# AutonomousVehicleLaboratory/vision_semantic_segmentation

Measured on AMD Instinct MI355X. Metric: fused frames/sec/GPU (1920x1080 + 120k pts) + max|dlog-odds| vs ref, higher is better.
Workload: dtype f16 hi+lo split, MX-FP4 correction passes, fp32 accumulate

## Files before the change

vision_semantic_segmentation_amd/csrc/seg_bottleneck.hip:

```cpp
#include "seg_types.h"

namespace avl {
namespace {

constexpr int BT_H = 8, BT_W = 16;
constexpr int BH_W = BT_W + 2, BH_H = BT_H + 2;
constexpr int BN_HALO = BH_W * BH_H;
constexpr int BN_M1 = 12;
constexpr int BN_WIDTH = 128, BN_COUT = 256;
constexpr int XSLAB = 192 * 128;
constexpr int PLANE1 = 192 * 256;
constexpr int PLANE2 = 128 * 256;

struct BnArgs {
    const f16* x;
    const f16* x_lo;
    f16* out;
    f16* out_lo;
    const f16* w1;
    const f16* w2;
    const f16* w3;
    const float* b1;
    const float* b2;
    const float* b3;
    int H, W, in_ld, out_ld;
    int tiles_x, ntiles;
    int out_bytes;
};

template <int CIN, bool DS, bool T1LO>
struct BnLayout {
    static constexpr int NCH = CIN / 64;
    static constexpr int XTILE = NCH * XSLAB;
    static constexpr int XBYTES = (DS ? 2 : 1) * XTILE;
    static constexpr int T1LO_OFF = PLANE1;
    static constexpr int T2LO_OFF = T1LO ? PLANE1 : PLANE2;
    static constexpr int ABYTES = T1LO ? 2 * PLANE1 : 2 * PLANE2;
    static constexpr int LDS = XBYTES + ABYTES;
    static_assert(LDS <= 160 * 1024, "bottleneck tile does not fit the LDS");
};

typedef f16 h2v __attribute__((ext_vector_type(2)));
typedef unsigned u32x4 __attribute__((ext_vector_type(4)));

__device__ __forceinline__ float relu_f32(float v) { return __builtin_amdgcn_fmed3f(v, 0.f, 3.0e38f); }

__device__ __forceinline__ uint2 relu_pack4(f32x4 v) {
    const h2v z = {(f16)0.f, (f16)0.f};
    const h2v a = __builtin_elementwise_max(h2v{(f16)v[0], (f16)v[1]}, z), b = __builtin_elementwise_max(h2v{(f16)v[2], (f16)v[3]}, z);
    return make_uint2(__builtin_bit_cast(unsigned, a), __builtin_bit_cast(unsigned, b));
}

__device__ __forceinline__ unsigned lo_pair(unsigned hipk, float v0, float v1) {
    unsigned d;
    asm("v_fma_mixlo_f16 %0, -%1, 1.0, %2 op_sel_hi:[1,0,0]" : "=v"(d) : "v"(hipk), "v"(v0));
    asm("v_fma_mixhi_f16 %0, -%1, 1.0, %2 op_sel:[1,0,0] op_sel_hi:[1,0,0]" : "+v"(d) : "v"(hipk), "v"(v1));
    return d;
}

__device__ __forceinline__ void split4(const float (&v)[4], uint2& hi, uint2& lo) {
    const h2v a = {(f16)v[0], (f16)v[1]}, b = {(f16)v[2], (f16)v[3]};
    hi = make_uint2(__builtin_bit_cast(unsigned, a), __builtin_bit_cast(unsigned, b));
    lo = make_uint2(lo_pair(hi.x, v[0], v[1]), lo_pair(hi.y, v[2], v[3]));
}

template <int CIN, bool DS, bool T1LO, bool XLO, bool OLO>
__global__ void __launch_bounds__(512) k_bottleneck(BnArgs p) {
    typedef BnLayout<CIN, DS, T1LO> L;
    constexpr int KS1 = CIN / 32;
    constexpr int KS3 = 4 + (DS ? CIN / 32 : 0);
    extern __shared__ __attribute__((aligned(16))) char lds[];
    const int tid = threadIdx.x, lane = tid & 63;
    const int wave = __builtin_amdgcn_readfirstlane(tid >> 6);
    const int c = lane & 15, q = lane >> 4;
    const unsigned lds0 = lds_addr(lds);
    char* const A = lds + L::XBYTES;
// ... 242 lines not shown
                    __builtin_amdgcn_raw_buffer_store_b128(u32x4{h0.x, h0.y, h1.x, h1.y}, orsrc, ooff, 0, 0);
                }
            }
        }
        {
            constexpr int NTAIL = (DS ? BT_H : BT_H - 2) * (OLO ? 2 : 1);
            if (more) asm volatile("s_waitcnt vmcnt(%0)" ::"n"(NTAIL) : "memory");
        }
        __syncthreads();
    }
}

int device_cus() {
    static int n = 0;
    if (n == 0) {
        int dev = 0;
        hipDeviceProp_t prop;
        if (hipGetDevice(&dev) == hipSuccess && hipGetDeviceProperties(&prop, dev) == hipSuccess) n = prop.multiProcessorCount;
        if (n <= 0) n = 256;
    }
    return n;
}

template <int CIN, bool DS, bool T1LO, bool XLO, bool OLO>
int launch_bn(const BnArgs& a, int nimg, hipStream_t s) {
    typedef BnLayout<CIN, DS, T1LO> L;
    AVL_HIP_CHECK(hipFuncSetAttribute(reinterpret_cast<const void*>(&k_bottleneck<CIN, DS, T1LO, XLO, OLO>), hipFuncAttributeMaxDynamicSharedMemorySize, L::LDS));
    const int grid = a.ntiles < device_cus() ? a.ntiles : device_cus();
    hipLaunchKernelGGL((k_bottleneck<CIN, DS, T1LO, XLO, OLO>), dim3(grid, 1, nimg), dim3(512), L::LDS, s, a);
    AVL_LAUNCH_CHECK();
    return AVL_OK;
}

}

int validate_bottleneck(const avl_seg_op& op) {
    AVL_REQUIRE(op.dtype == AVL_F16, "fused bottleneck: AVL_F16 activations only");
    AVL_REQUIRE(op.groups == 32 && op.ksize == 3 && op.stride == 1 && op.dil == 1 && op.pad == 1, "fused bottleneck: 3x3, 32 groups, stride 1, dilation 1");
    AVL_REQUIRE(op.out_c == BN_COUT && op.in3_c == BN_WIDTH, "fused bottleneck: width %d -> %d output channels only (got %d -> %d)", BN_WIDTH, BN_COUT, op.in3_c, op.out_c);
    AVL_REQUIRE((op.in_c == 64 && op.w_layout == 1) || (op.in_c == 256 && op.w_layout == 0 && op.w_split == 0),
                "fused bottleneck: 64 input channels with the downsample folded in, or 256 with the identity residual and no t1 lo plane");
    AVL_REQUIRE(op.in_h == op.out_h && op.in_w == op.out_w && op.in_h > 0 && op.in_w > 0, "fused bottleneck: same-size output");
    AVL_REQUIRE(op.in_ld >= op.in_c && op.in_ld % 8 == 0 && op.out_ld >= op.out_c && op.out_ld % 8 == 0, "fused bottleneck: row strides");
    AVL_REQUIRE((long long)op.in_rows >= (long long)op.in_h * op.in_w * op_batch(op) && (long long)op.out_rows >= (long long)op.out_h * op.out_w * op_batch(op),
                "fused bottleneck: rows allocated");
    AVL_REQUIRE((long long)op.in_rows * op.in_ld * 2 < (1LL << 31) && (long long)op.out_rows * op.out_ld * 2 < (1LL << 31), "fused bottleneck: planes beyond 2 GB (32-bit offsets)");
    AVL_REQUIRE(op.in && op.out && op.weight && op.in2 && op.in3 && op.bias, "fused bottleneck: in, out, weight (conv1), in2 (conv2 weights), in3 (conv3 weights), bias");
    AVL_REQUIRE(((reinterpret_cast<uintptr_t>(op.in) | reinterpret_cast<uintptr_t>(op.in_lo) | reinterpret_cast<uintptr_t>(op.out) | reinterpret_cast<uintptr_t>(op.out_lo) |
                  reinterpret_cast<uintptr_t>(op.weight) | reinterpret_cast<uintptr_t>(op.in2) | reinterpret_cast<uintptr_t>(op.in3) | reinterpret_cast<uintptr_t>(op.bias)) & 15) == 0,
                "fused bottleneck: 16-byte aligned buffers");
    AVL_REQUIRE(!(op.in_c == 64 && op.in_lo), "fused bottleneck: the 64-channel variant takes a single-plane input");
    AVL_REQUIRE(op.in != op.out && op.in != op.out_lo, "fused bottleneck: not in place (tiles read their neighbours' pixels)");
    return AVL_OK;
}

int launch_bottleneck(const avl_seg_op& op, hipStream_t s) {
    BnArgs a;
    a.x = static_cast<const f16*>(op.in);
    a.x_lo = static_cast<const f16*>(op.in_lo);
    a.out = static_cast<f16*>(op.out);
    a.out_lo = static_cast<f16*>(op.out_lo);
    a.w1 = static_cast<const f16*>(op.weight);
    a.w2 = static_cast<const f16*>(op.in2);
    a.w3 = static_cast<const f16*>(op.in3);
    a.b1 = op.bias; a.b2 = op.bias + BN_WIDTH; a.b3 = op.bias + 2 * BN_WIDTH;
    a.H = op.in_h; a.W = op.in_w; a.in_ld = op.in_ld; a.out_ld = op.out_ld;
    a.tiles_x = (op.in_w + BT_W - 1) / BT_W;
    a.ntiles = a.tiles_x * ((op.in_h + BT_H - 1) / BT_H);
    a.out_bytes = (int)((long long)op.out_rows * op.out_ld * 2);
    const int variant = (op.in_c == 64 ? 4 + 2 * (op.w_split ? 1 : 0) : 2 * (a.x_lo ? 1 : 0)) + (a.out_lo ? 1 : 0);
    switch (variant) {
        case 0: return launch_bn<256, false, false, false, false>(a, op_batch(op), s);
        case 1: return launch_bn<256, false, false, false, true>(a, op_batch(op), s);
        case 2: return launch_bn<256, false, false, true, false>(a, op_batch(op), s);
        case 3: return launch_bn<256, false, false, true, true>(a, op_batch(op), s);
        case 4: return launch_bn<64, true, false, false, false>(a, op_batch(op), s);
        case 5: return launch_bn<64, true, false, false, true>(a, op_batch(op), s);
        case 6: return launch_bn<64, true, true, false, false>(a, op_batch(op), s);
        default: return launch_bn<64, true, true, false, true>(a, op_batch(op), s);
    }
}

}
```

vision_semantic_segmentation_amd/csrc/seg_gemm.hip:

```cpp
#include <cstdlib>
#include <cstring>
#include <type_traits>

#include "seg_types.h"

namespace avl {
namespace {

struct GemmArgs {
    const void* A;
    const void* W;
    const float* bias;
    const void* R;
    void* C;
    int lda, ldr, ldc;
    int M, N, K;
    int relu, out_f32;
    int ntiles;
    int nsub;
    long long a_lo_delta;
    const void* R_lo;
    void* C_lo;
};

// ... 439 lines not shown
    constexpr int LDS = 2 * (WM * 64 + WN * 64) * 128;
    AVL_HIP_CHECK(hipFuncSetAttribute(reinterpret_cast<const void*>(&k_gemm<T, WM, WN>),
                                      hipFuncAttributeMaxDynamicSharedMemorySize, LDS));
    hipLaunchKernelGGL((k_gemm<T, WM, WN>), dim3(mtiles * a.ntiles), dim3(WM * WN * 64), LDS, s, a);
    AVL_LAUNCH_CHECK();
    return AVL_OK;
}

struct MxArgs {
    GemmArgs g;
    const char* Aq[2];
    const char* As[2];
    const char* Wq[2];
    const char* Ws[2];
    int ldaq;
    long long a_srows, w_srows;
    char* Cq[2];
    char* Cs[2];
    int ldcq;
    long long c_srows;
    int nmx;
    const char* Rq;
    const char* Rs;
    int ldrq;
    long long r_srows;
    int nmb1;
    const void* A2;
    int lda2, ldaq2;
    const char* Aq2[2];
    const char* As2[2];
    long long a_srows2;
    int stagger;
};

__device__ __forceinline__ unsigned quantize_fp4_block(const float (&v)[16], unsigned (&q)[2]) {
    float amax = 0.f;
#pragma unroll
    for (int i = 0; i < 16; ++i) amax = fmaxf(amax, fabsf(v[i]));
    {
        const unsigned ab = __float_as_uint(amax);
        const auto r16 = __builtin_amdgcn_permlane16_swap(ab, ab, false, false);
        amax = __uint_as_float(max(r16[0], r16[1]));
    }
    const unsigned sbyte = mx_fp4_scale_byte(amax);
    const float scale = __uint_as_float(sbyte << 23);
    q[0] = q[1] = 0u;
#define AVL_FP4_PAIR(i)                                                                                  \
    q[0] = __builtin_amdgcn_cvt_scalef32_pk_fp4_f32(q[0], v[2 * (i)], v[2 * (i) + 1], scale, (i));        \
    q[1] = __builtin_amdgcn_cvt_scalef32_pk_fp4_f32(q[1], v[8 + 2 * (i)], v[8 + 2 * (i) + 1], scale, (i))
    AVL_FP4_PAIR(0); AVL_FP4_PAIR(1); AVL_FP4_PAIR(2); AVL_FP4_PAIR(3);
#undef AVL_FP4_PAIR
    return sbyte;
}

template <int IO, int MI>
__device__ __forceinline__ void mx_epilogue(const MxArgs& q, f32x4 (&acc)[MI][4], int nt, int mt, int wm, int wn, int fr, int kq) {
    typedef f16 H;
    typedef typename Half16<H>::v8 v8;
    constexpr int BM = 2 * MI * 16, BN = 256;
    const GemmArgs& p = q.g;
    const int nbase = nt * BN + wn * 64 + kq * 16;
    const bool ncol_ok = nbase + 16 <= p.N;
    const bool rsplit = p.R_lo != nullptr, csplit = p.C_lo != nullptr;
    const unsigned m0 = (unsigned)(mt * BM + wm * (MI * 16) + fr);
    const unsigned sc_r = (unsigned)(nbase >> 8) * (unsigned)q.r_srows * 8u + (unsigned)((nbase >> 5) & 7);
    const unsigned sc_c = (unsigned)(nbase >> 8) * (unsigned)q.c_srows * 8u + (unsigned)((nbase >> 5) & 7);
    v8 nr0 = {}, nr1 = {};
    uint2 npk = make_uint2(0u, 0u);
    unsigned nsb = 127u;
    auto load_res = [&](int mi) {
        const unsigned m = m0 + mi * 16;
        if (p.R && (int)m < p.M && ncol_ok) {
            const H* rp = static_cast<const H*>(p.R) + (m * (unsigned)p.ldr + (unsigned)nbase);
            nr0 = *reinterpret_cast<const v8*>(rp);
            nr1 = *reinterpret_cast<const v8*>(rp + 8);
            if (q.Rq) {
                npk = *reinterpret_cast<const uint2*>(q.Rq + (m * (unsigned)q.ldrq + (unsigned)(nbase / 2)));
                nsb = (unsigned char)q.Rs[sc_r + m * 8u];
            }
        }
    };
    load_res(0);
#pragma unroll
    for (int mi = 0; mi < MI; ++mi) {
        const unsigned m = m0 + mi * 16;
        const bool live = (int)m < p.M && ncol_ok;
// ... 744 lines not shown
```

vision_semantic_segmentation_amd/csrc/seg_types.h:

```cpp
#pragma once
#include <hip/hip_runtime.h>

#include "avl_common.h"

namespace avl {

typedef __bf16 bf16;
typedef __bf16 bf16x8 __attribute__((ext_vector_type(8)));
typedef _Float16 f16;
typedef _Float16 f16x8 __attribute__((ext_vector_type(8)));
typedef float f32x4 __attribute__((ext_vector_type(4)));
typedef float f32x8 __attribute__((ext_vector_type(8)));

template <typename T>
struct Vec8;

template <>
struct Vec8<bf16> {
    static __device__ __forceinline__ void load(const bf16* p, float (&v)[8]) {
        const bf16x8 x = *reinterpret_cast<const bf16x8*>(p);
#pragma unroll
        for (int i = 0; i < 8; ++i) v[i] = (float)x[i];
    }
    static __device__ __forceinline__ void store(bf16* p, const float (&v)[8]) {
// ... 73 lines not shown
}

__device__ __forceinline__ void glds16_saddr(const void* sbase, unsigned voff, unsigned lds_byte_addr) {
    unsigned keep;
    asm volatile(
        "s_mov_b32 %0, m0\n\t"
        "s_mov_b32 m0, %3\n\t"
        "s_nop 0\n\t"
        "global_load_lds_dwordx4 %1, %2\n\t"
        "s_mov_b32 m0, %0"
        : "=&s"(keep)
        : "v"(voff), "s"(sbase), "s"(lds_byte_addr)
        : "memory");
}

__device__ __forceinline__ void glds4_saddr(const void* sbase, unsigned voff, unsigned lds_byte_addr) {
    unsigned keep;
    asm volatile(
        "s_mov_b32 %0, m0\n\t"
        "s_mov_b32 m0, %3\n\t"
        "s_nop 0\n\t"
        "global_load_lds_dword %1, %2\n\t"
        "s_mov_b32 m0, %0"
        : "=&s"(keep)
        : "v"(voff), "s"(sbase), "s"(lds_byte_addr)
        : "memory");
}

__device__ __forceinline__ unsigned mx_fp4_scale_byte(float amax) {
    const unsigned ab = __float_as_uint(amax), e = ab >> 23;
    return (e >= 3u ? e - 2u : 1u) + ((ab & 0x7fffffu) > 0x500000u ? 1u : 0u);
}

__device__ __forceinline__ unsigned lds_addr(const void* p) {
    return (unsigned)(size_t)(const __attribute__((address_space(3))) void*)p;
}

inline int elem_size(int dtype) { return dtype == AVL_F32 ? 4 : 2; }

inline int op_batch(const avl_seg_op& op) { return op.batch > 1 ? op.batch : 1; }
template <typename T>
__device__ __forceinline__ T* image_base(T* p, long long pixels, long long ld) {
    return p ? p + (long long)blockIdx.z * pixels * ld : p;
}
inline bool is_half(int dtype) { return dtype == AVL_BF16 || dtype == AVL_F16; }

int launch_gemm(const avl_seg_op& op, hipStream_t s);
int validate_gemm(const avl_seg_op& op);
int launch_conv_op(const avl_seg_op& op, hipStream_t s);
int validate_conv_op(const avl_seg_op& op);
int launch_gconv_mfma(const avl_seg_op& op, hipStream_t s);
int validate_gconv_mfma(const avl_seg_op& op);
int launch_conv3x3(const avl_seg_op& op, hipStream_t s);
int validate_conv3x3(const avl_seg_op& op);
int launch_stem_mfma(const avl_seg_op& op, hipStream_t s);
int launch_stem_pre_f32(const avl_seg_op& op, hipStream_t s);
int launch_dwconv_k(const avl_seg_op& op, hipStream_t s);
int validate_dwconv_k(const avl_seg_op& op);
int launch_dwpw(const avl_seg_op& op, hipStream_t s);
int validate_dwpw(const avl_seg_op& op);
int launch_bottleneck(const avl_seg_op& op, hipStream_t s);
int validate_bottleneck(const avl_seg_op& op);

}
```

vision_semantic_segmentation_amd/network.py:

```python
import ctypes as C
import math

import numpy as np
import torch

from . import _lib

BN_EPS = 1e-5

OP_STEM, OP_MAXPOOL, OP_GEMM, OP_GCONV, OP_DWCONV, OP_BILINEAR, OP_GAP, OP_GEMV, OP_ARGMAX, OP_SUBSAMPLE, OP_DWPW, OP_BOTTLENECK = range(1, 13)
OP_NAMES = {1: "stem", 2: "maxpool", 3: "gemm", 4: "gconv", 5: "dwconv", 6: "bilinear", 7: "gap", 8: "gemv", 9: "argmax", 10: "subsample", 11: "dwpw",
            12: "bottleneck"}


class AvlSegOp(C.Structure):
    _fields_ = [
        ("kind", C.c_int32), ("dtype", C.c_int32),
        ("in_", C.c_void_p), ("in2", C.c_void_p), ("out", C.c_void_p), ("weight", C.c_void_p), ("bias", C.c_void_p),
        ("in_h", C.c_int32), ("in_w", C.c_int32), ("in_c", C.c_int32), ("in_ld", C.c_int32), ("in_rows", C.c_int32),
        ("out_h", C.c_int32), ("out_w", C.c_int32), ("out_c", C.c_int32), ("out_ld", C.c_int32), ("out_rows", C.c_int32),
        ("in2_ld", C.c_int32),
        ("ksize", C.c_int32), ("stride", C.c_int32), ("pad", C.c_int32), ("dil", C.c_int32), ("groups", C.c_int32),
        ("relu", C.c_int32), ("out_f32", C.c_int32), ("w_rows", C.c_int32), ("w_layout", C.c_int32), ("w_split", C.c_int32), ("mx_flags", C.c_int32),
        ("in_lo", C.c_void_p), ("in2_lo", C.c_void_p), ("out_lo", C.c_void_p),
# ... 284 lines not shown
    order = [r * tx + c for b in range(0, ty, band) for c in range(tx) for r in range(b, min(b + band, ty))]
    return torch.tensor(order, dtype=torch.int32)


def _round_up(x, m):
    return (x + m - 1) // m * m


def split_f16(w):
    hi = w.to(torch.float16)
    lo = (w - hi.to(torch.float64)).to(torch.float16)
    return hi, lo


def pack_split_rows(w, nsub):
    rows, k = w.shape
    assert k % 64 == 0 and nsub in (2, 3)
    hi, lo = split_f16(w)
    parts = [hi.reshape(rows, k // 64, 1, 64), lo.reshape(rows, k // 64, 1, 64)]
    if nsub == 3:
        parts.append(parts[0])
    return torch.cat(parts, dim=2).reshape(rows, k * nsub).contiguous()


def _mfma_a_fragments(m):
    rows, k = m.shape
    return m.reshape(rows // 16, 16, k // 32, 4, 8).permute(0, 2, 3, 1, 4).reshape(rows // 16, k // 32, 64, 8)


def pack_bottleneck(w1, w2, w3, wd, groups):
    width, cin = w1.shape
    cout = w3.shape[0]
    cg = width // groups
    assert width % 16 == 0 and cin % 32 == 0 and cout % 32 == 0 and 16 % cg == 0

    def pair(m):
        hi, lo = split_f16(m)
        return torch.stack([_mfma_a_fragments(hi), _mfma_a_fragments(lo)], dim=2)

    p1 = pair(w1.to(torch.float64))
    nwin = width // 16
    dense = torch.zeros((nwin, 16, 10, 16), dtype=torch.float64)
    wt = w2.reshape(width, cg, 9).to(torch.float64)
    co = torch.arange(width)
    win, col = co // 16, co % 16
    gbase = (col // cg) * cg
    for ci in range(cg):
        dense[win, col, :9, gbase + ci] = wt[co, ci, :]
    p2 = pair(dense.reshape(nwin * 16, 160))
    w3k = w3.to(torch.float64) if wd is None else torch.cat([w3.to(torch.float64), wd.to(torch.float64)], dim=1)
    i = torch.arange(16)
    rows = torch.cat([32 * wv + (i >> 2) * 8 + nj * 4 + (i & 3) for wv in range(cout // 32) for nj in range(2)])
    p3 = pair(w3k[rows])
    ks3 = w3k.shape[1] // 32
    p3 = p3.reshape(cout // 32, 2, ks3, 2, 64, 8).permute(0, 2, 1, 3, 4, 5)
    return p1.reshape(-1).contiguous(), p2.reshape(-1).contiguous(), p3.reshape(-1).contiguous()


_FP4_GRID = torch.tensor([0.0, 0.5, 1.0, 1.5, 2.0, 3.0, 4.0, 6.0], dtype=torch.float64)


def fp4_quant_blocks(b):
    b = b.to(torch.float64)
    amax = b.abs().amax(dim=-1)
    e = (torch.floor(torch.log2(amax.clamp_min(2.0 ** -200))).to(torch.int64) + 127).clamp_min(0)
    sbyte = torch.where(e >= 3, e - 2, torch.ones_like(e))
    mant = amax.to(torch.float32).view(torch.int32).to(torch.int64) & 0x7FFFFF
    sbyte = (sbyte + (mant > 0x500000).to(torch.int64)).clamp(1, 254)
    scale = torch.exp2((sbyte - 127).to(torch.float64)).unsqueeze(-1)
    mag = (b.abs() / scale).clamp_max(6.0)
    mid = (_FP4_GRID[1:] + _FP4_GRID[:-1]) / 2
    code = torch.bucketize(mag, mid, right=False)
    tie = mag == mid[code.clamp(0, 6)]
    code = torch.where(tie & (code % 2 == 1), code + 1, code)
    code = code.clamp(0, 7) | ((b < 0).to(torch.int64) << 3)
    code = code.reshape(*code.shape[:-1], 16, 2)
    return (code[..., 0] | (code[..., 1] << 4)).to(torch.uint8), sbyte


def mx_quant_fp4(w):
    rows, k = w.shape
    assert k % 256 == 0
    packed, sbyte = fp4_quant_blocks(w.reshape(rows, k // 32, 32))
    scales = sbyte.reshape(rows, k // 256, 8).permute(1, 0, 2).contiguous().to(torch.uint8)
    return packed.reshape(rows, k // 2), scales


def mx_dequant_fp4(packed, scales):
# ... 271 lines not shown
                f.update(in2_mx=res.mx.data_ptr())
                flags |= AVL_MX_RES_LO
            if isinstance(dst, Act) and dst.mx is not None and dst_col == 0 and dst.hi.shape[1] == cout:
                f.update(out_mx=dst.mx.data_ptr())
                dst.mx_valid = True
                if dst.lo_fp4:
                    flags |= AVL_MX_OUT_LO
        else:
            for t_, what in ((src if read_lo else None, "input"), (res, "residual"), (dst, "output")):
                if isinstance(t_, Act) and t_.lo_fp4:
                    raise RuntimeError("%s: the %s keeps its lo part as FP4 only, which needs the MX GEMM" % (name, what))
        f["mx_flags"] = flags
        if labels is not None:
            assert out_f32 and not use_mx and res is None and not relu
            f["out_mx"] = labels.data_ptr()
        if bias_per_image and self.batch > 1:
            assert not use_mx and bias_dev.shape == (self.batch, w_rows)
            f["bias_per_image"] = 1
        self._op(name, OP_GEMM, **f)

    def _bottleneck(self, p, st, x, hw, cin, width, cout, y):
        w1, b1 = fold_bn(st, p + ".conv1.weight", p + ".bn1")
        w2, b2 = fold_bn(st, p + ".conv2.weight", p + ".bn2")
        w3, b3 = fold_bn(st, p + ".conv3.weight", p + ".bn3")
        wd = None
        if (p + ".downsample.0.weight") in st:
            wd, bd = fold_bn(st, p + ".downsample.0.weight", p + ".downsample.1")
            wd, b3 = wd.reshape(cout, cin), b3 + bd
        p1, p2, p3 = (self._dev(t, torch.float16) for t in _cached_pack(
            (self._fp, self.backbone, p, "bottleneck"), lambda: pack_bottleneck(w1.reshape(width, cin), w2, w3.reshape(cout, width), wd, self.groups)))
        bias = self._dev(torch.cat([b1, b2, b3]), torch.float32)
        ip, ild, irows = self._view(x)
        op_, old, orows = self._view(y)
        self._op(p, OP_BOTTLENECK, in_=ip, in_lo=self._lo(x), out=op_, out_lo=self._lo(y), weight=p1.data_ptr(), in2=p2.data_ptr(), in3=p3.data_ptr(),
                 in3_c=width, bias=bias.data_ptr(), in_h=hw[0], in_w=hw[1], in_c=cin, in_ld=ild, in_rows=irows, out_h=hw[0], out_w=hw[1],
                 out_c=cout, out_ld=old, out_rows=orows, ksize=3, stride=1, pad=1, dil=1, groups=self.groups, relu=1, w_layout=int(wd is not None),
                 w_split=int(wd is not None))

    def _dwpw(self, name, src, hw, cin, w_dw, b_dw, w_pw, b_pw, dst, dst_col, dilation, padding=None, classifier=None):
        h, wd = hw
        padding = dilation if padding is None else padding
        oh, ow = h + 2 * padding - 2 * dilation, wd + 2 * padding - 2 * dilation
        cout = w_pw.shape[0]
        w_rows = _round_up(cout, 256)
        wp = torch.zeros((w_rows, cin), dtype=torch.float64)
        wp[:cout] = w_pw.reshape(cout, cin)
        bp = torch.zeros(w_rows, dtype=torch.float64)
        bp[:cout] = b_pw
        wdev = self._dev(pack_split_rows(wp, 2), torch.float16) if self.mixed else self._dev(wp, self.act_dtype)
        bdev = self._dev(bp, torch.float32)
        exact = self.mixed and self.mixed_dw_exact
        in_lo = self._lo(src) if exact else 0
        dwp = pack_dw_f32(w_dw, b_dw) if exact else pack_dw_pairs(w_dw, b_dw, self.act_dtype)
        blocks = bool(in_lo) and dilation == 1
        params = torch.cat([dwp, dwpw_block_order(oh, ow) if blocks else dwpw_tile_order(oh, ow, dilation)]).to(self.device)
        self._keep.append(params)
        ip, ild, irows = self._view(src)
        if classifier is not None:
            wc, bc, logits, labels = classifier
            ncls = wc.shape[0]
            assert in_lo and cout == 256 and ncls <= 32 and wc.shape[1] == cout
            wc32 = torch.zeros((32, cout), dtype=torch.float64)
            wc32[:ncls] = wc
            bc32 = torch.zeros(32, dtype=torch.float64)
            bc32[:ncls] = bc
            wcd = self._dev(torch.stack(split_f16(wc32)), torch.float16)
            bcd = self._dev(bc32, torch.float32)
# ... 61 lines not shown
        x = self._act(h4 * w4, 64, split=self.full_split)
        self._spatial("backbone.maxpool", OP_MAXPOOL, stem, (h2, w2), 64, x, (h4, w4), 64, ksize=3, stride=2, pad=1, dil=1,
                      **(dict(in_lo=self._lo(stem), out_lo=self._lo(x)) if self.full_split else {}))
        self._release(stem)

        hw, cin = (h4, w4), 64
        dilation = 1
        low = None
        dilated = (False, False, True, True) if self.output_stride == 8 else (False, False, False, True)
        groups = self.groups
        for li, (planes, nblocks, stride0, dilate) in enumerate(zip(PLANES, self.layers, (1, 2, 2, 2), dilated), start=1):
            width = int(planes * (self.width_per_group / 64.0)) * groups
            cg = width // groups
            dense = cg % 64 == 0
            assert dense or (cg <= 32 and 32 % cg == 0), "%s: %d channels per group" % (self.backbone, cg)
            cout = planes * EXPANSION
            previous_dilation = dilation
            stride = stride0
            if dilate:
                dilation *= stride
                stride = 1
            for bi in range(nblocks):
                p = "backbone.layer%d.%d" % (li, bi)
                trunk_lo = self.mixed_layer1_lo or li != 1 or bi == nblocks - 1
                s = stride if bi == 0 else 1
                d = previous_dilation if bi == 0 else dilation
                ohw = ((hw[0] + 2 * d - 2 * d - 1) // s + 1, (hw[1] + 2 * d - 2 * d - 1) // s + 1)
                if (self.mixed_fuse_block and s == 1 and d == 1 and width == 128 and cout == 256 and cin in (64, 256) and groups == 32 and 16 % cg == 0
                        and ((p + ".downsample.0.weight") in st) == (cin == 64) and x.hi.shape[1] == cin and (cin == 256 or x.lo is None)):
                    y = self._act(ohw[0] * ohw[1], cout, split=trunk_lo)
                    self._bottleneck(p, st, x, hw, cin, width, cout, y)
                    if x is not low:
                        self._release(x)
                    x, hw, cin = y, ohw, cout
                    continue
                w, b = fold_bn(st, p + ".conv1.weight", p + ".bn1")
                conv1_mx = (self.mixed_mx and self.mixed_gconv_mx and x.mx is not None and x.mx_valid and x.hi.shape[1] == cin
                            and cin % 256 == 0 and width % 256 == 0 and not dense and 32 % cg == 0)
                t1_c = _round_up(width, 128) if self.full_split else width
                if t1_c != width:
                    w = torch.cat([w, torch.zeros((t1_c - width,) + tuple(w.shape[1:]), dtype=w.dtype)])
                    b = torch.cat([b, torch.zeros(t1_c - width, dtype=b.dtype)])
                t1 = self._act(hw[0] * hw[1], t1_c, split=self.full_split, mx=conv1_mx, lo_fp4=conv1_mx)
                self._gemm(p + ".conv1", x, hw, cin, w, b, t1, read_lo=self.mixed_conv1_split)
                w, b = fold_bn(st, p + ".conv2.weight", p + ".bn2")
                gconv_mx = self.mixed and t1.mx is not None and t1.mx_valid and t1.lo_fp4 and not dense
                wsplit = int(self.mixed)
                extra_g = {}
                if dense:
                    if self.mixed:
                        wg_d = self._dev(_cached_pack((self._fp, self.backbone, p + ".conv2", "dense_split"),
                                                      lambda: pack_conv3x3(w, groups, 8, split=True)), torch.float16)
                    else:
                        wg_d = self._dev(_cached_pack((self._fp, self.backbone, p + ".conv2", "dense", self.half),
                                                      lambda: pack_conv3x3(w, groups, 8 if self.half else 4)), self.act_dtype)
                    layout = 2
                elif gconv_mx:
                    frag_hi, bundle = _cached_pack((self._fp, self.backbone, p + ".conv2", "gconv_mx"), lambda: pack_gconv_mx(w, groups))
                    wg_d, layout, wsplit = self._dev(frag_hi.reshape(-1), torch.float16), 1, 2
                    wb = bundle.to(self.device)
                    self._keep.append(wb)
                    extra_g = dict(w_mx=wb.data_ptr(), in_mx=t1.mx.data_ptr(), mx_flags=AVL_MX_IN_LO)
                elif self.half and width % 64 == 0 and 32 % cg == 0:
                    if self.mixed:
                        nwin = width // 32
                        whi, wlo = split_f16(w)
# ... 323 lines not shown
```

Baseline: 226.8.

## Fuse layer2 512-channel bottleneck blocks into one MX-aware kernel

Adds a fused bottleneck kernel for the layer2 identity blocks (512 in, width 256, 512 out). It chains conv1, the grouped 3x3 conv2 and conv3 plus the residual inside LDS per 4x16 tile, with a three-slab input ring. The kernel reads and writes the MX-FP4 lo-correction trunk directly, so the separate conv GEMMs and their intermediate global round trips go away. The trade-offs are a new large-LDS kernel with heavy register use, an fp16 overflow flag path, and new weight-packing logic for cout 512.

```diff
diff --git a/vision_semantic_segmentation_amd/csrc/seg_bottleneck.hip b/vision_semantic_segmentation_amd/csrc/seg_bottleneck.hip
--- a/vision_semantic_segmentation_amd/csrc/seg_bottleneck.hip
+++ b/vision_semantic_segmentation_amd/csrc/seg_bottleneck.hip
@@ -42,6 +42,7 @@
 
 typedef f16 h2v __attribute__((ext_vector_type(2)));
 typedef unsigned u32x4 __attribute__((ext_vector_type(4)));
+typedef unsigned u32x2 __attribute__((ext_vector_type(2)));
 
 __device__ __forceinline__ float relu_f32(float v) { return __builtin_amdgcn_fmed3f(v, 0.f, 3.0e38f); }
 
@@ -350,11 +351,331 @@
     return AVL_OK;
 }
 
+constexpr int B2_TH = 4, B2_TW = 16;
+constexpr int B2_HW = B2_TW + 2, B2_HH = B2_TH + 2;
+constexpr int B2_HALO = B2_HW * B2_HH;
+constexpr int B2_M1 = 7;
+constexpr int B2_CIN = 512, B2_WIDTH = 256, B2_COUT = 512;
+constexpr int B2_NSLAB = B2_CIN / 64;
+constexpr int B2_SLAB = 128 * 128;
+constexpr int B2_RING = 3 * B2_SLAB;
+constexpr int B2_T1 = B2_RING;
+constexpr int B2_T2LO = B2_T1 + 112 * 512;
+constexpr int B2_FLAG = B2_T2LO + 64 * 512;
+constexpr int B2_LDS = B2_FLAG + 16;
+static_assert(B2_LDS <= 160 * 1024, "layer2 bottleneck tile does not fit the LDS");
+
+struct Bn2Args {
+    const f16* x;
+    const char* xq;
+    f16* out;
+    char* oq;
+    const f16* w1;
+    const f16* w2;
+    const f16* w3;
+    const float* b;
+    int H, W, in_ld, out_ld;
+    int tiles_x, ntiles;
+    int in_rows, out_rows;
+};
+
+__global__ void __launch_bounds__(512) k_bottleneck_w256(Bn2Args p) {
+    extern __shared__ __attribute__((aligned(16))) char lds[];
+    const int tid = threadIdx.x, lane = tid & 63;
+    const int wave = __builtin_amdgcn_readfirstlane(tid >> 6);
+    const int c = lane & 15, q = lane >> 4;
+    const unsigned lds0 = lds_addr(lds);
+    char* const T1 = lds + B2_T1;
+    char* const T2L = lds + B2_T2LO;
+    const int ipix = p.H * p.W;
+    const int row0 = (int)blockIdx.z * ipix;
+
+    int bid = blockIdx.x;
+    {
+        const int nwg = gridDim.x, xcd = bid & 7, local = bid >> 3, qq = nwg >> 3, r = nwg & 7;
+        bid = (xcd < r ? xcd * (qq + 1) : r * (qq + 1) + (xcd - r) * qq) + local;
+    }
+
+    auto stage = [&](int tile, int s) __attribute__((always_inline)) {
+        const int ty = tile / p.tiles_x, tx = tile - ty * p.tiles_x;
+        int lo_ = lane;
+        asm volatile("" : "+v"(lo_));
+#pragma unroll
+        for (int j = 0; j < 2; ++j) {
+            const int gi = wave + 8 * j;
+            const int pix = gi * 8 + (lo_ >> 3);
+            const int hy = min(pix / B2_HW, B2_HH - 1), hx = pix - (pix / B2_HW) * B2_HW;
+            const int iy = min(max(ty * B2_TH - 1 + hy, 0), p.H - 1), ix = min(max(tx * B2_TW - 1 + hx, 0), p.W - 1);
+            const unsigned voff = ((unsigned)(row0 + iy * p.W + ix) * (unsigned)p.in_ld + (unsigned)(s * 64) + (unsigned)(((lo_ & 7) ^ (pix & 7)) << 3)) * 2u;
+            glds16_saddr(p.x, voff, lds0 + (s % 3) * B2_SLAB + gi * 1024);
+        }
+    };
+
+    const __amdgpu_buffer_rsrc_t w1r = __builtin_amdgcn_make_buffer_rsrc(const_cast<char*>(reinterpret_cast<const char*>(p.w1)) + (size_t)wave * (2 * 16 * 2 * 1024), 0, 2 * 16 * 2 * 1024, 0x00020000);
+    const __amdgpu_buffer_rsrc_t w3r = __builtin_amdgcn_make_buffer_rsrc(const_cast<char*>(reinterpret_cast<const char*>(p.w3)) + (size_t)wave * (8 * 4 * 2 * 1024), 0, 8 * 4 * 2 * 1024, 0x00020000);
+    const int wlane = lane * 16;
+    auto wfrag = [&](__amdgpu_buffer_rsrc_t r, int frag) __attribute__((always_inline)) {
+        return __builtin_bit_cast(f16x8, __builtin_amdgcn_raw_buffer_load_b128(r, wlane + frag * 1024, 0, 0));
+    };
+    auto load_w1 = [&](int s, f16x8 (&wf)[2][2][2]) __attribute__((always_inline)) {
+#pragma unroll
+        for (int nt = 0; nt < 2; ++nt)
+#pragma unroll
+            for (int kk = 0; kk < 2; ++kk)
+#pragma unroll
+                for (int hl = 0; hl < 2; ++hl) wf[nt][kk][hl] = wfrag(w1r, (nt * 16 + 2 * s + kk) * 2 + hl);
+    };
+
+    const unsigned x_rd = (unsigned)(c * 128) + (unsigned)((q ^ (c & 7)) << 4);
+    const int ch0 = 64 * wave + 16 * q;
+
+    int tile = bid;
+    volatile int* const ovf = reinterpret_cast<volatile int*>(lds + B2_FLAG);
+    f16x8 w1f[2][2][2][2];
+    if (tile < p.ntiles) { stage(tile, 0); stage(tile, 1); load_w1(0, w1f[0]); }
+
+    for (; tile < p.ntiles; tile += gridDim.x) {
+        const int ty = tile / p.tiles_x, tx = tile - ty * p.tiles_x;
+        int co = c, qo = q;
+        asm volatile("" : "+v"(co), "+v"(qo));
+        const bool more = tile + (int)gridDim.x < p.ntiles;
+
+        f32x4 acc1[B2_M1][2];
+#pragma unroll
+        for (int nt = 0; nt < 2; ++nt) {
+            const float4 b = *reinterpret_cast<const float4*>(p.b + 16 * (2 * wave + nt) + 4 * qo);
+#pragma unroll
+            for (int m = 0; m < B2_M1; ++m) acc1[m][nt] = f32x4{b.x, b.y, b.z, b.w};
+        }
+        f16x8 w2f[2][5][2];
+#pragma unroll
+        for (int s = 0; s < B2_NSLAB; ++s) {
+            if (s == 0 || s + 1 >= B2_NSLAB) asm volatile("s_waitcnt vmcnt(0)" ::: "memory");
+            else asm volatile("s_waitcnt vmcnt(2)" ::: "memory");
+            __syncthreads();
+            if (s == 0 && tid == 0) *ovf = 0;
+            if (s + 1 < B2_NSLAB) load_w1(s + 1, w1f[(s + 1) & 1]);
+            else {
+                const f16x8* w2p = reinterpret_cast<const f16x8*>(p.w2 + (size_t)wave * (2 * 5 * 2 * 512)) + (co + 16 * qo);
+#pragma unroll
+                for (int j = 0; j < 2; ++j)
+#pragma unroll
+                    for (int k2 = 0; k2 < 5; ++k2) { w2f[j][k2][0] = w2p[(j * 5 + k2) * 128]; w2f[j][k2][1] = w2p[(j * 5 + k2) * 128 + 64]; }
+            }
+            if (s + 2 < B2_NSLAB) stage(tile, s + 2);
+            const char* X = lds + (s % 3) * B2_SLAB;
+            f16x8 xf[2][2];
+            auto read_x = [&](int m, f16x8 (&f)[2]) __attribute__((always_inline)) {
+                f[0] = *reinterpret_cast<const f16x8*>(X + x_rd + m * 2048);
+                f[1] = *reinterpret_cast<const f16x8*>(X + (x_rd ^ 64u) + m * 2048);
+            };
+            read_x(0, xf[0]);
+#pragma unroll
+            for (int m = 0; m < B2_M1; ++m) {
+                if (m + 1 < B2_M1) read_x(m + 1, xf[(m + 1) & 1]);
+#pragma unroll
+                for (int kk = 0; kk < 2; ++kk)
+#pragma unroll
+                    for (int nt = 0; nt < 2; ++nt) {
+                        acc1[m][nt] = __builtin_amdgcn_mfma_f32_16x16x32_f16(w1f[s & 1][nt][kk][0], xf[m & 1][kk], acc1[m][nt], 0, 0, 0);
+                        acc1[m][nt] = __builtin_amdgcn_mfma_f32_16x16x32_f16(w1f[s & 1][nt][kk][1], xf[m & 1][kk], acc1[m][nt], 0, 0, 0);
+                    }
+            }
+        }
+        unsigned hmax = 0u;
+#pragma unroll
+        for (int m = 0; m < B2_M1; ++m) {
+            const int h = m * 16 + co;
+            const int hy = h / B2_HW, hx = h - hy * B2_HW;
+            const int iy = ty * B2_TH - 1 + hy, ix = tx * B2_TW - 1 + hx;
+            const bool valid = ((unsigned)(h < B2_HALO) & (unsigned)((unsigned)iy < (unsigned)p.H) & (unsigned)((unsigned)ix < (unsigned)p.W)) != 0u;
+            const unsigned vm = valid ? 0xffffffffu : 0u;
+#pragma unroll
+            for (int nt = 0; nt < 2; ++nt) {
+                const int n = 2 * wave + nt;
+                const uint2 hi = relu_pack4(acc1[m][nt]);
+                hmax = max(hmax, max(max((hi.x & vm) & 0xffffu, (hi.x & vm) >> 16), max((hi.y & vm) & 0xffffu, (hi.y & vm) >> 16)));
+                const unsigned off = (unsigned)(h * 512) + (unsigned)((((2 * n) | (qo >> 1)) ^ co) << 4) + (unsigned)((qo & 1) * 8);
+                *reinterpret_cast<uint2*>(T1 + off) = make_uint2(hi.x & vm, hi.y & vm);
+            }
+        }
+#pragma unroll
+        for (int j = 0; j < 2; ++j) {
+            const int n = 2 * wave + j;
+            const float4 bias2 = *reinterpret_cast<const float4*>(p.b + B2_WIDTH + 16 * n + 4 * qo);
+            const unsigned cw16 = (unsigned)(((2 * n) | (qo & 1)) << 4);
+#pragma unroll
+            for (int r = 0; r < B2_TH; ++r) {
+                f32x4 acc = f32x4{bias2.x, bias2.y, bias2.z, bias2.w};
+                f16x8 th[5];
+#pragma unroll
+                for (int ks = 0; ks < 5; ++ks) {
+                    const int t = min(2 * ks + (qo >> 1), 8);
+                    const unsigned h = (unsigned)((r + t / 3) * B2_HW + (t % 3) + co);
+                    th[ks] = *reinterpret_cast<const f16x8*>(T1 + (h << 9) + (cw16 ^ ((h & 15u) << 4)));
+                }
+                __builtin_amdgcn_sched_barrier(0);
+#pragma unroll
+                for (int ks = 0; ks < 5; ++ks) {
+                    acc = __builtin_amdgcn_mfma_f32_16x16x32_f16(w2f[j][ks][0], th[ks], acc, 0, 0, 0);
+                    acc = __builtin_amdgcn_mfma_f32_16x16x32_f16(w2f[j][ks][1], th[ks], acc, 0, 0, 0);
+                }
+                float v[4];
+#pragma unroll
+                for (int k = 0; k < 4; ++k) v[k] = relu_f32(acc[k]);
+                uint2 hi, lo;
+                split4(v, hi, lo);
+                const unsigned px = (unsigned)(r * 16 + co);
+                const unsigned off = (px << 9) + (unsigned)((((2 * n) | (qo >> 1)) ^ co) << 4) + (unsigned)((qo & 1) * 8);
+                *reinterpret_cast<uint2*>(T1 + off) = hi;
+                *reinterpret_cast<uint2*>(T2L + off) = lo;
+            }
+        }
+        if (hmax >= 0x7c00u) *ovf = 1;
+        __syncthreads();
+
+        if (more) { stage(tile + gridDim.x, 0); stage(tile + gridDim.x, 1); }
+
+        f32x4 acc3[B2_TH][4];
+#pragma unroll
+        for (int nj = 0; nj < 4; ++nj) {
+            const float4 b = *reinterpret_cast<const float4*>(p.b + 2 * B2_WIDTH + ch0 + 4 * nj);
+#pragma unroll
+            for (int r = 0; r < B2_TH; ++r) acc3[r][nj] = f32x4{b.x, b.y, b.z, b.w};
+        }
+        f16x8 w3f[2][4][2];
+        auto load_w3 = [&](int ks, f16x8 (&wf)[4][2]) __attribute__((always_inline)) {
+#pragma unroll
+            for (int nj = 0; nj < 4; ++nj) { wf[nj][0] = wfrag(w3r, (ks * 4 + nj) * 2); wf[nj][1] = wfrag(w3r, (ks * 4 + nj) * 2 + 1); }
+        };
+        uint4 resh[B2_TH][2];
+        uint2 resq[B2_TH];
+        unsigned ress[B2_TH];
+        auto load_res = [&]() __attribute__((always_inline)) {
+            const long long P = (long long)p.in_rows * (B2_CIN / 2), S = (long long)(B2_CIN / 256) * p.in_rows * 8;
+            const char* const rq = p.xq + P + S;
+            const unsigned char* const rs = reinterpret_cast<const unsigned char*>(p.xq + 2 * P + S);
+#pragma unroll
+            for (int r = 0; r < B2_TH; ++r) {
+                const unsigned grow = (unsigned)(row0 + min(ty * B2_TH + r, p.H - 1) * p.W + min(tx * B2_TW + co, p.W - 1));
+                resh[r][0] = *reinterpret_cast<const uint4*>(p.x + (grow * (unsigned)p.in_ld + (unsigned)ch0));
+                resh[r][1] = *reinterpret_cast<const uint4*>(p.x + (grow * (unsigned)p.in_ld + (unsigned)ch0 + 8u));
+                resq[r] = *reinterpret_cast<const uint2*>(rq + (grow * (unsigned)(B2_CIN / 2) + (unsigned)(ch0 / 2)));
+                ress[r] = rs[(unsigned)(ch0 >> 8) * (unsigned)p.in_rows * 8u + grow * 8u + (unsigned)((ch0 >> 5) & 7)];
+            }
+        };
+        load_res();
+        load_w3(0, w3f[0]);
+#pragma unroll
+        for (int ks = 0; ks < 8; ++ks) {
+            if (ks + 1 < 8) load_w3(ks + 1, w3f[(ks + 1) & 1]);
+            f16x8 th[B2_TH], tl[B2_TH];
+#pragma unroll
+            for (int r = 0; r < B2_TH; ++r) {
+                const unsigned off = (unsigned)((r * 16 + co) << 9) + (unsigned)((((4 * ks) + qo) ^ co) << 4);
+                th[r] = *reinterpret_cast<const f16x8*>(T1 + off);
+                tl[r] = *reinterpret_cast<const f16x8*>(T2L + off);
+            }
+#pragma unroll
+            for (int r = 0; r < B2_TH; ++r)
+#pragma unroll
+                for (int nj = 0; nj < 4; ++nj) {
+                    acc3[r][nj] = __builtin_amdgcn_mfma_f32_16x16x32_f16(w3f[ks & 1][nj][0], th[r], acc3[r][nj], 0, 0, 0);
+                    acc3[r][nj] = __builtin_amdgcn_mfma_f32_16x16x32_f16(w3f[ks & 1][nj][1], th[r], acc3[r][nj], 0, 0, 0);
+                    acc3[r][nj] = __builtin_amdgcn_mfma_f32_16x16x32_f16(w3f[ks & 1][nj][0], tl[r], acc3[r][nj], 0, 0, 0);
+                }
+        }
+        if (more) load_w1(0, w1f[0]);
+
+        const unsigned OP = (unsigned)p.out_rows * (B2_COUT / 2), OS = (unsigned)(B2_COUT / 256) * (unsigned)p.out_rows * 8u;
+#pragma unroll
+        for (int r = 0; r < B2_TH; ++r) {
+            const int oy = ty * B2_TH + r, ox = tx * B2_TW + co;
+            const bool live = ((unsigned)(oy < p.H) & (unsigned)(ox < p.W)) != 0u;
+            const unsigned grow = (unsigned)(row0 + min(oy, p.H - 1) * p.W + min(ox, p.W - 1));
+            const uint4 rh0 = resh[r][0], rh1 = resh[r][1];
+            const uint2 pk = resq[r];
+            const unsigned sb = ress[r];
+            float v[16];
+#pragma unroll
+            for (int nj = 0; nj < 4; ++nj)
+#pragma unroll
+                for (int k = 0; k < 4; ++k) v[nj * 4 + k] = acc3[r][nj][k];
+            {
+                const f16x8 h0 = __builtin_bit_cast(f16x8, rh0), h1 = __builtin_bit_cast(f16x8, rh1);
+                float rl[16];
+                typedef float v2f __attribute__((ext_vector_type(2)));
+                const float sc = __uint_as_float(sb << 23);
+#define AVL_FP4_DEC(w, sel, o) { const v2f d = __builtin_amdgcn_cvt_scalef32_pk_f32_fp4(w, sc, sel); rl[o] = d.x; rl[o + 1] = d.y; }
+                AVL_FP4_DEC(pk.x, 0, 0) AVL_FP4_DEC(pk.x, 1, 2) AVL_FP4_DEC(pk.x, 2, 4) AVL_FP4_DEC(pk.x, 3, 6)
+                AVL_FP4_DEC(pk.y, 0, 8) AVL_FP4_DEC(pk.y, 1, 10) AVL_FP4_DEC(pk.y, 2, 12) AVL_FP4_DEC(pk.y, 3, 14)
+#undef AVL_FP4_DEC
+#pragma unroll
+                for (int i = 0; i < 8; ++i) { v[i] += (float)h0[i] + rl[i]; v[8 + i] += (float)h1[i] + rl[8 + i]; }
+            }
+            float hi[16], lo[16];
+            unsigned hp[8];
+#pragma unroll
+            for (int i = 0; i < 16; i += 2) {
+                const float a = relu_f32(v[i]), b = relu_f32(v[i + 1]);
+                const h2v hh = {(f16)a, (f16)b};
+                hp[i / 2] = __builtin_bit_cast(unsigned, hh);
+                hi[i] = (float)hh[0]; hi[i + 1] = (float)hh[1];
+                lo[i] = a - hi[i]; lo[i + 1] = b - hi[i + 1];
+            }
+            unsigned q0[2], q1[2];
+            const unsigned s0 = quantize_fp4_block(hi, q0), s1 = quantize_fp4_block(lo, q1);
+            const unsigned ovm = *ovf != 0 ? 0x7c007c00u : 0u;
+#pragma unroll
+            for (int k = 0; k < 8; ++k) hp[k] |= ovm;
+            if (live) {
+                *reinterpret_cast<uint4*>(p.out + (grow * (unsigned)p.out_ld + (unsigned)ch0)) = make_uint4(hp[0], hp[1], hp[2], hp[3]);
+                *reinterpret_cast<uint4*>(p.out + (grow * (unsigned)p.out_ld + (unsigned)ch0 + 8u)) = make_uint4(hp[4], hp[5], hp[6], hp[7]);
+                const unsigned qoff = grow * (unsigned)(B2_COUT / 2) + (unsigned)(ch0 / 2);
+                *reinterpret_cast<uint2*>(p.oq + qoff) = make_uint2(q0[0], q0[1]);
+                *reinterpret_cast<uint2*>(p.oq + (qoff + OP + OS)) = make_uint2(q1[0], q1[1]);
+                if ((qo & 1) == 0) {
+                    const unsigned soff = (unsigned)(ch0 >> 8) * (unsigned)p.out_rows * 8u + grow * 8u + (unsigned)((ch0 >> 5) & 7);
+                    p.oq[OP + soff] = (char)s0;
+                    p.oq[2u * OP + OS + soff] = (char)s1;
+                }
+            }
+        }
+    }
+}
+
+int launch_bn2(const Bn2Args& a, int nimg, hipStream_t s) {
+    AVL_HIP_CHECK(hipFuncSetAttribute(reinterpret_cast<const void*>(&k_bottleneck_w256), hipFuncAttributeMaxDynamicSharedMemorySize, B2_LDS));
+    const int grid = a.ntiles < device_cus() ? a.ntiles : device_cus();
+    hipLaunchKernelGGL(k_bottleneck_w256, dim3(grid, 1, nimg), dim3(512), B2_LDS, s, a);
+    AVL_LAUNCH_CHECK();
+    return AVL_OK;
+}
+
+}
+
+static int validate_bottleneck_w256(const avl_seg_op& op) {
+    AVL_REQUIRE(op.out_c == B2_COUT && op.in3_c == B2_WIDTH && op.w_layout == 0 && op.w_split == 0,
+                "fused bottleneck (512 channels): width %d -> %d output channels, identity residual (got %d -> %d)", B2_WIDTH, B2_COUT, op.in3_c, op.out_c);
+    AVL_REQUIRE(op.in_mx && op.out_mx && !op.in_lo && !op.out_lo && op.mx_flags == (AVL_MX_IN_LO | AVL_MX_OUT_LO),
+                "fused bottleneck (512 channels): MX trunk in and out (in_mx, out_mx, mx_flags AVL_MX_IN_LO | AVL_MX_OUT_LO, no f16 lo planes)");
+    AVL_REQUIRE(op.in_ld == B2_CIN && op.out_ld == B2_COUT, "fused bottleneck (512 channels): dense rows (the bundles have no row stride)");
+    AVL_REQUIRE((long long)op.in_rows >= (long long)op.in_h * op.in_w * op_batch(op) && (long long)op.out_rows >= (long long)op.out_h * op.out_w * op_batch(op),
+                "fused bottleneck: rows allocated");
+    AVL_REQUIRE((long long)op.in_rows * op.in_ld * 2 < (1LL << 31) && (long long)op.out_rows * op.out_ld * 2 < (1LL << 31), "fused bottleneck: planes beyond 2 GB (32-bit offsets)");
+    AVL_REQUIRE(op.in && op.out && op.weight && op.in2 && op.in3 && op.bias, "fused bottleneck: in, out, weight (conv1), in2 (conv2 weights), in3 (conv3 weights), bias");
+    AVL_REQUIRE(((reinterpret_cast<uintptr_t>(op.in) | reinterpret_cast<uintptr_t>(op.out) | reinterpret_cast<uintptr_t>(op.in_mx) | reinterpret_cast<uintptr_t>(op.out_mx) |
+                  reinterpret_cast<uintptr_t>(op.weight) | reinterpret_cast<uintptr_t>(op.in2) | reinterpret_cast<uintptr_t>(op.in3) | reinterpret_cast<uintptr_t>(op.bias)) & 15) == 0,
+                "fused bottleneck: 16-byte aligned buffers");
+    AVL_REQUIRE(op.in != op.out && op.in_mx != op.out_mx, "fused bottleneck: not in place (tiles read their neighbours' pixels)");
+    return AVL_OK;
 }
 
 int validate_bottleneck(const avl_seg_op& op) {
     AVL_REQUIRE(op.dtype == AVL_F16, "fused bottleneck: AVL_F16 activations only");
     AVL_REQUIRE(op.groups == 32 && op.ksize == 3 && op.stride == 1 && op.dil == 1 && op.pad == 1, "fused bottleneck: 3x3, 32 groups, stride 1, dilation 1");
+    AVL_REQUIRE(op.in_h == op.out_h && op.in_w == op.out_w && op.in_h > 0 && op.in_w > 0, "fused bottleneck: same-size output");
+    if (op.in_c == B2_CIN) return validate_bottleneck_w256(op);
     AVL_REQUIRE(op.out_c == BN_COUT && op.in3_c == BN_WIDTH, "fused bottleneck: width %d -> %d output channels only (got %d -> %d)", BN_WIDTH, BN_COUT, op.in3_c, op.out_c);
     AVL_REQUIRE((op.in_c == 64 && op.w_layout == 1) || (op.in_c == 256 && op.w_layout == 0 && op.w_split == 0),
                 "fused bottleneck: 64 input channels with the downsample folded in, or 256 with the identity residual and no t1 lo plane");
@@ -373,6 +694,22 @@
 }
 
 int launch_bottleneck(const avl_seg_op& op, hipStream_t s) {
+    if (op.in_c == B2_CIN) {
+        Bn2Args a;
+        a.x = static_cast<const f16*>(op.in);
+        a.xq = static_cast<const char*>(op.in_mx);
+        a.out = static_cast<f16*>(op.out);
+        a.oq = static_cast<char*>(op.out_mx);
+        a.w1 = static_cast<const f16*>(op.weight);
+        a.w2 = static_cast<const f16*>(op.in2);
+        a.w3 = static_cast<const f16*>(op.in3);
+        a.b = op.bias;
+        a.H = op.in_h; a.W = op.in_w; a.in_ld = op.in_ld; a.out_ld = op.out_ld;
+        a.tiles_x = (op.in_w + B2_TW - 1) / B2_TW;
+        a.ntiles = a.tiles_x * ((op.in_h + B2_TH - 1) / B2_TH);
+        a.in_rows = op.in_rows; a.out_rows = op.out_rows;
+        return launch_bn2(a, op_batch(op), s);
+    }
     BnArgs a;
     a.x = static_cast<const f16*>(op.in);
     a.x_lo = static_cast<const f16*>(op.in_lo);
diff --git a/vision_semantic_segmentation_amd/csrc/seg_gemm.hip b/vision_semantic_segmentation_amd/csrc/seg_gemm.hip
--- a/vision_semantic_segmentation_amd/csrc/seg_gemm.hip
+++ b/vision_semantic_segmentation_amd/csrc/seg_gemm.hip
@@ -495,26 +495,6 @@
     long long a_srows2;
     int stagger;
 };
-
-__device__ __forceinline__ unsigned quantize_fp4_block(const float (&v)[16], unsigned (&q)[2]) {
-    float amax = 0.f;
-#pragma unroll
-    for (int i = 0; i < 16; ++i) amax = fmaxf(amax, fabsf(v[i]));
-    {
-        const unsigned ab = __float_as_uint(amax);
-        const auto r16 = __builtin_amdgcn_permlane16_swap(ab, ab, false, false);
-        amax = __uint_as_float(max(r16[0], r16[1]));
-    }
-    const unsigned sbyte = mx_fp4_scale_byte(amax);
-    const float scale = __uint_as_float(sbyte << 23);
-    q[0] = q[1] = 0u;
-#define AVL_FP4_PAIR(i)                                                                                  \
-    q[0] = __builtin_amdgcn_cvt_scalef32_pk_fp4_f32(q[0], v[2 * (i)], v[2 * (i) + 1], scale, (i));        \
-    q[1] = __builtin_amdgcn_cvt_scalef32_pk_fp4_f32(q[1], v[8 + 2 * (i)], v[8 + 2 * (i) + 1], scale, (i))
-    AVL_FP4_PAIR(0); AVL_FP4_PAIR(1); AVL_FP4_PAIR(2); AVL_FP4_PAIR(3);
-#undef AVL_FP4_PAIR
-    return sbyte;
-}
 
 template <int IO, int MI>
 __device__ __forceinline__ void mx_epilogue(const MxArgs& q, f32x4 (&acc)[MI][4], int nt, int mt, int wm, int wn, int fr, int kq) {
diff --git a/vision_semantic_segmentation_amd/csrc/seg_types.h b/vision_semantic_segmentation_amd/csrc/seg_types.h
--- a/vision_semantic_segmentation_amd/csrc/seg_types.h
+++ b/vision_semantic_segmentation_amd/csrc/seg_types.h
@@ -129,6 +129,26 @@
     return (e >= 3u ? e - 2u : 1u) + ((ab & 0x7fffffu) > 0x500000u ? 1u : 0u);
 }
 
+__device__ __forceinline__ unsigned quantize_fp4_block(const float (&v)[16], unsigned (&q)[2]) {
+    float amax = 0.f;
+#pragma unroll
+    for (int i = 0; i < 16; ++i) amax = fmaxf(amax, fabsf(v[i]));
+    {
+        const unsigned ab = __float_as_uint(amax);
+        const auto r16 = __builtin_amdgcn_permlane16_swap(ab, ab, false, false);
+        amax = __uint_as_float(max(r16[0], r16[1]));
+    }
+    const unsigned sbyte = mx_fp4_scale_byte(amax);
+    const float scale = __uint_as_float(sbyte << 23);
+    q[0] = q[1] = 0u;
+#define AVL_FP4_PAIR(i)                                                                                  \
+    q[0] = __builtin_amdgcn_cvt_scalef32_pk_fp4_f32(q[0], v[2 * (i)], v[2 * (i) + 1], scale, (i));        \
+    q[1] = __builtin_amdgcn_cvt_scalef32_pk_fp4_f32(q[1], v[8 + 2 * (i)], v[8 + 2 * (i) + 1], scale, (i))
+    AVL_FP4_PAIR(0); AVL_FP4_PAIR(1); AVL_FP4_PAIR(2); AVL_FP4_PAIR(3);
+#undef AVL_FP4_PAIR
+    return sbyte;
+}
+
 __device__ __forceinline__ unsigned lds_addr(const void* p) {
     return (unsigned)(size_t)(const __attribute__((address_space(3))) void*)p;
 }
diff --git a/vision_semantic_segmentation_amd/network.py b/vision_semantic_segmentation_amd/network.py
--- a/vision_semantic_segmentation_amd/network.py
+++ b/vision_semantic_segmentation_amd/network.py
@@ -340,7 +340,7 @@
     width, cin = w1.shape
     cout = w3.shape[0]
     cg = width // groups
-    assert width % 16 == 0 and cin % 32 == 0 and cout % 32 == 0 and 16 % cg == 0
+    assert width % 16 == 0 and cin % 32 == 0 and cout in (256, 512) and 16 % cg == 0
 
     def pair(m):
         hi, lo = split_f16(m)
@@ -358,10 +358,11 @@
     p2 = pair(dense.reshape(nwin * 16, 160))
     w3k = w3.to(torch.float64) if wd is None else torch.cat([w3.to(torch.float64), wd.to(torch.float64)], dim=1)
     i = torch.arange(16)
-    rows = torch.cat([32 * wv + (i >> 2) * 8 + nj * 4 + (i & 3) for wv in range(cout // 32) for nj in range(2)])
+    nj_ = cout // 128
+    rows = torch.cat([16 * nj_ * wv + (i >> 2) * 4 * nj_ + nj * 4 + (i & 3) for wv in range(8) for nj in range(nj_)])
     p3 = pair(w3k[rows])
     ks3 = w3k.shape[1] // 32
-    p3 = p3.reshape(cout // 32, 2, ks3, 2, 64, 8).permute(0, 2, 1, 3, 4, 5)
+    p3 = p3.reshape(8, nj_, ks3, 2, 64, 8).permute(0, 2, 1, 3, 4, 5)
     return p1.reshape(-1).contiguous(), p2.reshape(-1).contiguous(), p3.reshape(-1).contiguous()
 
 
@@ -699,7 +700,11 @@
         bias = self._dev(torch.cat([b1, b2, b3]), torch.float32)
         ip, ild, irows = self._view(x)
         op_, old, orows = self._view(y)
-        self._op(p, OP_BOTTLENECK, in_=ip, in_lo=self._lo(x), out=op_, out_lo=self._lo(y), weight=p1.data_ptr(), in2=p2.data_ptr(), in3=p3.data_ptr(),
+        mx = {}
+        if cin == 512:
+            mx = dict(in_mx=x.mx.data_ptr(), out_mx=y.mx.data_ptr(), mx_flags=AVL_MX_IN_LO | AVL_MX_OUT_LO)
+            y.mx_valid = True
+        self._op(p, OP_BOTTLENECK, **mx, in_=ip, in_lo=self._lo(x), out=op_, out_lo=self._lo(y), weight=p1.data_ptr(), in2=p2.data_ptr(), in3=p3.data_ptr(),
                  in3_c=width, bias=bias.data_ptr(), in_h=hw[0], in_w=hw[1], in_c=cin, in_ld=ild, in_rows=irows, out_h=hw[0], out_w=hw[1],
                  out_c=cout, out_ld=old, out_rows=orows, ksize=3, stride=1, pad=1, dil=1, groups=self.groups, relu=1, w_layout=int(wd is not None),
                  w_split=int(wd is not None))
@@ -827,6 +832,14 @@
                     self._bottleneck(p, st, x, hw, cin, width, cout, y)
                     if x is not low:
                         self._release(x)
+                    x, hw, cin = y, ohw, cout
+                    continue
+                if (self.mixed_fuse_block and li == 2 and bi > 0 and s == 1 and d == 1 and width == 256 and cout == 512 and cin == 512
+                        and groups == 32 and cg == 8 and (p + ".downsample.0.weight") not in st and x.hi.shape[1] == cin and x.lo is None
+                        and x.mx is not None and x.mx_valid and x.lo_fp4):
+                    y = self._act(ohw[0] * ohw[1], cout, split=True, mx=True, lo_fp4=True)
+                    self._bottleneck(p, st, x, hw, cin, width, cout, y)
+                    self._release(x)
                     x, hw, cin = y, ohw, cout
                     continue
                 w, b = fold_bn(st, p + ".conv1.weight", p + ".bn1")
```

After: 230.3, median of 6. 1.02x the previous value.
